# tarepan/VectorQuantizedCPC

Hardware: AMD Instinct MI355X
Metric: audio samples/sec (WaveRNN-style decode, convert.py path: encode + generate) (higher is better)
Workload: dtype f32

## Files before the change

### vectorquantizedcpc_amd/csrc/scan.hip

```cpp
#include "common.h"
#include "ar_shared.h"
#include <math.h>

__global__ void build_wfrag_kernel(const float *__restrict__ W, int ldw, float *__restrict__ Wf, int n_rg,
                                   int K, int ksplit, int rowmode, int H) {
    const int SW = K / 16 / ksplit;
    const size_t total = (size_t)n_rg * ksplit * SW * 64;
    const size_t id = (size_t)blockIdx.x * blockDim.x + threadIdx.x;
    if (id >= total) return;
    const int lane = (int)(id & 63);
    size_t r = id >> 6;
    const int s = (int)(r % SW); r /= SW;
    const int w = (int)(r % ksplit);
    const int rg = (int)(r / ksplit);
    const int i = lane & 15, kq = lane >> 4, S = w * SW + s;
    int row;
    if (rowmode == 0) row = 16 * rg + i;
    else if (rowmode == 8) row = i < 8 ? 8 * rg + i : -1;
    else if (rowmode == 16) row = (rg % 3) * H + 16 * (rg / 3) + i;
    else row = (i >> 2) < rowmode ? (i >> 2) * H + 4 * rg + (i & 3) : -1;
    float4 v = make_float4(0.f, 0.f, 0.f, 0.f);
    if (row >= 0) v = *(const float4 *)(W + (size_t)row * ldw + 16 * S + 4 * kq);
    ((float4 *)Wf)[id] = v;
}
// ... 56 lines not shown
    float4 wf[SW];
    load_wfrag<SW>(p.Wf + (size_t)dir * (H / 4) * (H / 16) * 64 * 4, rg, 4, wave, lane, wf);
    const f32x4 acc = mv16<SW>(wf, hin, H, bt, wave, lane);
    const float v = reduce4(red, acc, wave, lane, tid);
    gate[tid >> 4][tid & 15] = v;
    __syncthreads();
    if (act) {
        float hn;
        if (G == 3) {
            const float r = sigmoidf_(g0 + (gate[u][b] + bh0));
            const float z = sigmoidf_(g1 + (gate[4 + u][b] + bh1));
            const float n = tanhf(g2 + r * (gate[8 + u][b] + bh2));
            hn = (1.0f - z) * n + z * hold;
        } else {
            const float ig = sigmoidf_(g0 + gate[u][b]), fg = sigmoidf_(g1 + gate[4 + u][b]);
            const float gg = tanhf(g2 + gate[8 + u][b]), og = sigmoidf_(g3 + gate[12 + u][b]);
            const float cn = fg * cold + ig * gg;
            p.cbuf[(size_t)dir * hsz + hi] = cn;
            hn = og * tanhf(cn);
        }
        hout[hi] = hn;
        p.out[((p.row0 ? (size_t)p.row0[bg] : (size_t)bg * p.T) + tpos) * (p.ndir * H) + (size_t)dir * H + unit] = hn;
    }
}

template <int G>
static int launch_seq(const SeqP &p, int step, hipStream_t s) {
    const int SW = p.H / 64;
    dim3 grid(p.H / 4, p.ndir, p.nbt), blk(256);
    switch (SW) {
#define CASE(n) case n: hipLaunchKernelGGL((seq_step_kernel<G, n>), grid, blk, 0, s, p, step); break;
        CASE(1) CASE(2) CASE(4) CASE(8)
#undef CASE
        default: vq_set_error("recurrent step: hidden size %d unsupported (64, 128, 256 and 512 are built)", p.H); return VQCPC_ERR_INVALID;
    }
    return VQCPC_OK;
}

int vq_bigru_scan(const float *Wf, const float *b_hh, const float *Gi, float *hbuf, float *out, const int *len, const int *row0,
                  int H, int B, int T, hipStream_t s) {
    const int nbt = (B + 15) / 16;
    HIP_TRY(hipMemsetAsync(hbuf, 0, (size_t)2 * 2 * nbt * H * 16 * sizeof(float), s));
    SeqP q{};
    q.Wf = Wf; q.b_hh = b_hh; q.Gi = Gi; q.hbuf = hbuf;
    q.out = out; q.len = len; q.row0 = row0; q.H = H; q.nbt = nbt; q.B = B; q.T = T; q.ndir = 2;
    for (int t = 0; t < T; ++t) TRY(launch_seq<3>(q, t, s));
    return VQCPC_OK;
}

__global__ void add_vec_kernel(const float *a, const float *b, float *o, int n) {
    const int i = blockIdx.x * blockDim.x + threadIdx.x;
    if (i < n) o[i] = a[i] + b[i];
}

struct LstmPlan {
    int D, H;
    float *w_ih = nullptr, *bias = nullptr, *Wf = nullptr;
    float *w_hh = nullptr;
    DevBuf gi, hbuf, cbuf, px;
    unsigned *abort_host = nullptr;
    int persistent = -1;
    bool pending = false;
    int dbg_drop_step = -1;
    int timeout_ms = 1000;
};
static int lstm_persist_launch(LstmPlan *p, int T, float *out, hipStream_t s);
void vq_lstm_plan_destroy(LstmPlan *p) {
    if (!p) return;
    if (p->w_ih) (void)hipFree(p->w_ih);
    if (p->bias) (void)hipFree(p->bias);
    if (p->Wf) (void)hipFree(p->Wf);
    if (p->w_hh) (void)hipFree(p->w_hh);
    if (p->abort_host) (void)hipHostFree(p->abort_host);
    p->gi.release(); p->hbuf.release(); p->cbuf.release(); p->px.release();
    delete p;
}
int vq_lstm_plan_create(const float *w_ih, const float *w_hh, const float *b_ih, const float *b_hh, int D, int H,
                        LstmPlan **out) {
    VQ_REQUIRE(D % 32 == 0 && (H == 64 || H == 128 || H == 256 || H == 512), "LSTM: need D %% 32 == 0 and a hidden size of 64, 128, 256 "
               "(model.py:57) or 512 (got %d, %d)", D, H);
    LstmPlan *p = new LstmPlan();
    p->D = D; p->H = H;
    *out = p;
    HIP_TRY(hipMalloc((void **)&p->w_ih, (size_t)4 * H * D * sizeof(float)));
    HIP_TRY(hipMemcpy(p->w_ih, w_ih, (size_t)4 * H * D * sizeof(float), hipMemcpyDeviceToDevice));
    HIP_TRY(hipMalloc((void **)&p->bias, (size_t)4 * H * sizeof(float)));
    hipLaunchKernelGGL(add_vec_kernel, dim3((4 * H + 255) / 256), dim3(256), 0, 0, b_ih, b_hh, p->bias, 4 * H);
    HIP_TRY(hipGetLastError());
    TRY(vq_build_wfrag(w_hh, H, H / 4, H, 4, 4, H, &p->Wf));
    HIP_TRY(hipMalloc((void **)&p->w_hh, (size_t)4 * H * H * sizeof(float)));
    HIP_TRY(hipMemcpy(p->w_hh, w_hh, (size_t)4 * H * H * sizeof(float), hipMemcpyDeviceToDevice));
    HIP_TRY(hipHostMalloc((void **)&p->abort_host, 64, hipHostMallocMapped));
    *p->abort_host = 0u;
    return VQCPC_OK;
}
int vq_lstm_set_persistent(LstmPlan *p, int value) { p->persistent = value; return VQCPC_OK; }
int vq_lstm_set_debug(LstmPlan *p, int drop_step, int timeout_ms) { p->dbg_drop_step = drop_step; p->timeout_ms = timeout_ms; return VQCPC_OK; }
int vq_lstm_check(LstmPlan *p) {
    if (!p->pending) return VQCPC_OK;
    p->pending = false;
    if (*(volatile unsigned *)p->abort_host != 0u) {
        *p->abort_host = 0u;
        p->persistent = 0;
        vq_set_error("encoder LSTM: an in-kernel exchange of the resident scan timed out (the context of that call is incomplete); "
                     "this handle now uses one launch per time step -- call again");
        return VQCPC_ERR_HIP;
    }
    return VQCPC_OK;
}
int vq_lstm_run(LstmPlan *p, const float *x, int B, int T, float *out, hipStream_t s) {
    const int H = p->H, nbt = (B + 15) / 16;
    TRY(p->gi.reserve((size_t)B * T * 4 * H * sizeof(float)));
    const size_t hsz = (size_t)nbt * H * 16 * sizeof(float);
    TRY(p->hbuf.reserve(2 * hsz));
    TRY(p->cbuf.reserve(hsz));
    TRY(vq_gemm_chain(x, p->D, p->w_ih, p->bias, p->gi.as<float>(), 4 * H, B * T, 4 * H, p->D, p->D, s));
    TRY(vq_lstm_check(p));
    if (p->persistent != 0 && B == 1 && H == 256 && T >= 1) return lstm_persist_launch(p, T, out, s);
    HIP_TRY(hipMemsetAsync(p->hbuf.p, 0, 2 * hsz, s));
    HIP_TRY(hipMemsetAsync(p->cbuf.p, 0, hsz, s));
    SeqP q{};
    q.Wf = p->Wf; q.Gi = p->gi.as<float>(); q.hbuf = p->hbuf.as<float>(); q.cbuf = p->cbuf.as<float>();
    q.out = out; q.len = nullptr; q.H = H; q.nbt = nbt; q.B = B; q.T = T; q.ndir = 1;
    for (int t = 0; t < T; ++t) TRY(launch_seq<4>(q, t, s));
    HIP_TRY(hipGetLastError());
    return VQCPC_OK;
}

__device__ __forceinline__ int ps_perm(int k) { return (k & ~15) | ((k & 3) << 2) | ((k >> 2) & 3); }

template <int NS>
__device__ __forceinline__ float ps_chain(const float (&w)[8 * NS], const float4 *hb, int kw, int c0) {
    float acc = 0.f;
#pragma unroll
    for (int s = 0; s < NS; ++s) {
        const float4 h0 = hb[(kw * NS + s) * 4 + c0], h1 = hb[(kw * NS + s) * 4 + c0 + 2];
        acc = __builtin_fmaf(w[8 * s + 0], h0.x, acc); acc = __builtin_fmaf(w[8 * s + 1], h0.y, acc);
        acc = __builtin_fmaf(w[8 * s + 2], h0.z, acc); acc = __builtin_fmaf(w[8 * s + 3], h0.w, acc);
        acc = __builtin_fmaf(w[8 * s + 4], h1.x, acc); acc = __builtin_fmaf(w[8 * s + 5], h1.y, acc);
        acc = __builtin_fmaf(w[8 * s + 6], h1.z, acc); acc = __builtin_fmaf(w[8 * s + 7], h1.w, acc);
    }
    return acc;
}
__device__ __forceinline__ float ps_combine(float acc, int lane) {
    (void)lane;
    const float other = PS_DPP(acc, 0xB1);
    const float q = acc + other;
    const float q1 = PS_DPP(q, 0x4E);
    const float q2 = PS_DPP(q, 0x104);
    const float q3 = PS_DPP(q, 0x106);
    return ((q + q1) + q2) + q3;
}

#define PS_PAD 16
__device__ __forceinline__ int ps_slot(int idx, int per_blk) { return (idx / per_blk) * PS_PAD + idx % per_blk; }

template <int N>
__device__ __forceinline__ bool ps_sweep(const u64 *g, int lane, int per_blk, unsigned tag, unsigned (&val)[N], unsigned *abort_flag,
                                         u64 ticks = 100000000ull) {
    const u64 t0 = __builtin_amdgcn_s_memrealtime();
    int slot[N];
#pragma unroll
    for (int j = 0; j < N; ++j) slot[j] = ps_slot(lane + 64 * j, per_blk);
    for (unsigned spins = 0;; ++spins) {
        bool ok = true;
#pragma unroll
        for (int j = 0; j < N; ++j) {
            const u64 x = ps_load(g + slot[j]);
            val[j] = (unsigned)x;
            ok &= (unsigned)(x >> 32) == tag;
        }
        if (__all(ok)) return true;
        if ((spins & 63) == 63) {
            const bool late = __builtin_amdgcn_s_memrealtime() - t0 > ticks;
            if (late || __hip_atomic_load(abort_flag, __ATOMIC_RELAXED, __HIP_MEMORY_SCOPE_SYSTEM) != 0u) {
                if (late && lane == 0) __hip_atomic_store(abort_flag, 1u, __ATOMIC_RELAXED, __HIP_MEMORY_SCOPE_SYSTEM);
                return false;
            }
        }
        __builtin_amdgcn_s_sleep(1);
    }
}

#define LP_NW 32
#define LP_UPB 8
struct LstmPersistP {
    const float *w_hh;
    const float *Gi;
    float *out;
    u64 *g;
    unsigned *abort_flag;
    int T;
    int force_agent;
    int dbg_drop_step;
    unsigned timeout_ticks;
};
template <bool LOCAL>
__device__ __forceinline__ void lp_store(u64 *p, u64 v) {
    if (LOCAL) asm volatile("global_store_dwordx2 %0, %1, off sc0" :: "v"(p), "v"(v) : "memory");
    else ps_store(p, v);
}
__global__ __launch_bounds__(256) void lstm_persist_kernel(LstmPersistP p) {
    constexpr int H = 256;
    if (blockIdx.x % 8 != 0) return;
    const int blk = blockIdx.x / 8, tid = threadIdx.x, lane = tid & 63, wave = tid >> 6;
    __shared__ __attribute__((aligned(16))) float hbuf[H];
    __shared__ float gsum[4 * LP_UPB];
    const int row_local = tid >> 3, gate = row_local / LP_UPB, ul = row_local % LP_UPB;
    const int kw = (lane & 7) >> 1, c0 = lane & 1;
    float w[8 * 4];
    ps_load_weights<4>(p.w_hh + (size_t)(gate * H + LP_UPB * blk + ul) * H, kw, c0, w);
    const int unit = LP_UPB * blk + (tid < LP_UPB ? tid : 0);
    const u64 *gw = p.g + (size_t)(8 * wave) * PS_PAD;
    unsigned xcc;
    asm volatile("s_getreg_b32 %0, hwreg(HW_REG_XCC_ID)" : "=s"(xcc));
    xcc &= 0xfu;
    if (tid == 0) ps_store(p.g + (size_t)blk * PS_PAD + 8, ((u64)0xC0DEu << 32) | xcc);
    bool dead = false, local = true;
    {
        const u64 t0 = __builtin_amdgcn_s_memrealtime();
        for (unsigned spins = 0;; ++spins) {
            const u64 x = ps_load(p.g + (size_t)(lane & 31) * PS_PAD + 8);
            if (__all((unsigned)(x >> 32) == 0xC0DEu)) { local = __all((unsigned)x == xcc) && !p.force_agent; break; }
            if ((spins & 63) == 63 && (__builtin_amdgcn_s_memrealtime() - t0 > 100000000ull ||
                                       __hip_atomic_load(p.abort_flag, __ATOMIC_RELAXED, __HIP_MEMORY_SCOPE_SYSTEM) != 0u)) {
                if (lane == 0) __hip_atomic_store(p.abort_flag, 1u, __ATOMIC_RELAXED, __HIP_MEMORY_SCOPE_SYSTEM);
                dead = true;
                break;
            }
            __builtin_amdgcn_s_sleep(1);
        }
    }
    float cst = 0.f;
    float gi0 = 0.f, gi1 = 0.f, gi2 = 0.f, gi3 = 0.f;
    if (tid < LP_UPB) { const float *gp = p.Gi + unit; gi0 = gp[0]; gi1 = gp[H]; gi2 = gp[2 * H]; gi3 = gp[3 * H]; }
    for (int t = 0; t < p.T; ++t) {
        float hv = 0.f;
        if (t > 0 && !dead) {
            unsigned v[1];
            if (ps_sweep<1>(gw + (size_t)((t - 1) & 1) * LP_NW * PS_PAD, lane, LP_UPB, (unsigned)t, v, p.abort_flag, (u64)p.timeout_ticks)) hv = __uint_as_float(v[0]);
            else dead = true;
        }
        hbuf[ps_perm(tid)] = hv;
        ps_barrier();
        const float acc = ps_chain<4>(w, (const float4 *)hbuf, kw, c0);
        const float v = ps_combine(acc, lane);
        if ((lane & 7) == 0) gsum[row_local] = v;
        ps_barrier();
        if (tid < LP_UPB) {
            const float ig = sigmoidf_(gi0 + gsum[tid]), fg = sigmoidf_(gi1 + gsum[LP_UPB + tid]);
            const float gg = tanhf(gi2 + gsum[2 * LP_UPB + tid]), og = sigmoidf_(gi3 + gsum[3 * LP_UPB + tid]);
            cst = fg * cst + ig * gg;
            const float hn = og * tanhf(cst);
            const u64 gr = ((u64)(unsigned)(t + 1) << 32) | __float_as_uint(hn);
            u64 *dst = p.g + ((size_t)(t & 1) * LP_NW + blk) * PS_PAD + tid;
            const bool drop = p.dbg_drop_step == t && blk == 3;
            if (drop) { }
            else if (local) lp_store<true>(dst, gr);
            else lp_store<false>(dst, gr);
            p.out[(size_t)t * H + unit] = hn;
            if (t + 1 < p.T) { const float *gp = p.Gi + (size_t)(t + 1) * 4 * H + unit; gi0 = gp[0]; gi1 = gp[H]; gi2 = gp[2 * H]; gi3 = gp[3 * H]; }
        }
    }
}
static int lstm_persist_launch(LstmPlan *p, int T, float *out, hipStream_t s) {
    const size_t bytes = (size_t)2 * LP_NW * PS_PAD * sizeof(u64);
    TRY(p->px.reserve(bytes));
    HIP_TRY(hipMemsetAsync(p->px.p, 0, bytes, s));
    LstmPersistP q{};
    q.w_hh = p->w_hh; q.Gi = p->gi.as<float>(); q.out = out; q.g = p->px.as<u64>(); q.T = T;
    q.force_agent = p->persistent == 2;
    q.dbg_drop_step = p->dbg_drop_step;
    q.timeout_ticks = (unsigned)p->timeout_ms * 100000u;
    HIP_TRY(hipHostGetDevicePointer((void **)&q.abort_flag, p->abort_host, 0));
    hipLaunchKernelGGL(lstm_persist_kernel, dim3(8 * LP_NW), dim3(256), 0, s, q);
    HIP_TRY(hipGetLastError());
    p->pending = true;
    return VQCPC_OK;
}
```

### vectorquantizedcpc_amd/csrc/vocoder_host.hip

```cpp
#include "vocoder_internal.h"
#include <math.h>
#include <stdio.h>
#include <limits.h>


__global__ void quads_build_kernel(const float *__restrict__ src, float4 *__restrict__ dst, int rows, int H) {
    const size_t id = (size_t)blockIdx.x * blockDim.x + threadIdx.x;
    if (id >= (size_t)rows * H) return;
    const int unit = (int)(id % H);
    const size_t row = id / H;
    const float *s = src + row * 3 * H + unit;
    dst[row * H + unit] = make_float4(s[0], s[H], s[2 * H], 0.f);
}

__global__ void glue_kernel(const int64_t *__restrict__ idx, const int64_t *__restrict__ spk,
                            const float *__restrict__ ce, const float *__restrict__ se, float *__restrict__ out,
                            int B, int Tc, int dz, int ds, int n_codes, int n_spk, unsigned *status, unsigned status_tag,
                            const int *__restrict__ frames, const int *__restrict__ row0) {
    const int F = dz + ds;
    size_t i = (size_t)blockIdx.x * blockDim.x + threadIdx.x;
    if (i >= (size_t)B * 2 * Tc * F) return;
    const int f = (int)(i % F);
    const size_t r = i / F;
    const int t2 = (int)(r % (2 * Tc)), b = (int)(r / (2 * Tc));
    if (row0) {
        if (t2 >= frames[b]) return;
        i = ((size_t)row0[b] + t2) * F + f;
    }
    if (f < dz) {
        long long z = idx[(size_t)b * Tc + t2 / 2];
        if ((z < 0 || z >= n_codes) && f == 0 && status) __hip_atomic_fetch_or(status, status_tag | STATUS_BAD_INDEX, __ATOMIC_RELAXED, __HIP_MEMORY_SCOPE_SYSTEM);
        z = z < 0 ? 0 : (z >= n_codes ? n_codes - 1 : z);
        out[i] = ce[(size_t)z * dz + f];
    } else {
        long long sp = spk[b];
        if ((sp < 0 || sp >= n_spk) && f == dz && t2 == 0 && status) __hip_atomic_fetch_or(status, status_tag | STATUS_BAD_INDEX, __ATOMIC_RELAXED, __HIP_MEMORY_SCOPE_SYSTEM);
        sp = sp < 0 ? 0 : (sp >= n_spk ? n_spk - 1 : sp);
        out[i] = se[(size_t)sp * ds + (f - dz)];
    }
}

__global__ void copy_submatrix_kernel(const float *__restrict__ src, int ld, int col0, float *__restrict__ dst,
                                      int rows, int cols) {
    const size_t i = (size_t)blockIdx.x * blockDim.x + threadIdx.x;
    if (i >= (size_t)rows * cols) return;
    const int r = (int)(i / cols), cidx = (int)(i % cols);
    dst[i] = src[(size_t)r * ld + col0 + cidx];
}
static ArStep step_of(vqcpc_vocoder *v) { return ArStep{v->d.Hr, v->d.Hf, v->d.n_cls, v->big_min_tiles, &v->big_attr_set}; }

static void clear_graphs(vqcpc_vocoder::Group &G) {
    for (auto &kv : G.graphs) (void)hipGraphExecDestroy(kv.second);
    G.graphs.clear();
}
static void clear_graphs(vqcpc_vocoder *v) {
    for (auto &G : v->grp) clear_graphs(G);
}

static std::vector<DevBuf *> device_buffers(vqcpc_vocoder *v, bool fixed) {
    std::vector<DevBuf *> b = {&v->series, &v->gi, &v->out0, &v->cond, &v->gcond, &v->gbase, &v->hseq, &v->len, &v->hall, &v->a1c, &v->nll_part, &v->nll_len,
                               &v->xd_x, &v->xd_segs};
    for (auto &G : v->grp) b.insert(b.end(), {&G.har, &G.a1, &G.cand_s, &G.cand_k, &G.slot_tab, &G.cur, &G.gcur, &G.candg});
    if (!fixed) return b;
    b.insert(b.end(), {&v->code_emb, &v->spk_emb, &v->w_cond, &v->b_ih, &v->Gemb, &v->Gemb4, &v->bh4, &v->Wf_hh12, &v->Wf_hh16, &v->b_hh, &v->Wf_fc1,
                       &v->Wf_fc1h, &v->b_fc1, &v->Wf_fc2, &v->b_fc2, &v->w_fc1, &v->w_fc2, &v->mulaw_tab, &v->w_hh, &v->grp[0].call, &v->grp[1].call});
    for (int l = 0; l < 2; ++l) b.insert(b.end(), {&v->p_wih[l], &v->p_bih[l], &v->p_bhh[l], &v->p_wf[l]});
    return b;
}

static int dcopy(DevBuf &dst, const float *src, size_t n) {
    TRY(dst.reserve(n * sizeof(float)));
    HIP_TRY(hipMemcpy(dst.p, src, n * sizeof(float), hipMemcpyDeviceToDevice));
    return VQCPC_OK;
}

extern "C" void vqcpc_vocoder_destroy(vqcpc_vocoder *v) {
    if (!v) return;
    clear_graphs(v);
    for (DevBuf *b : device_buffers(v, true)) b->release();
    v->stage.release();
    if (v->status_host) (void)hipHostFree(v->status_host);
    for (hipStream_t st : {v->side_stream, v->cap_stream}) if (st) (void)hipStreamDestroy(st);
    for (hipEvent_t e : {v->ev_fork, v->ev_join, v->ev0, v->ev1}) if (e) (void)hipEventDestroy(e);
    delete v;
}

static int vocoder_create_impl(const vqcpc_vocoder_weights *w, vqcpc_vocoder *v) {
    v->d = *w;
    const int F = w->dz + w->ds, Hp = w->Hp, dl = 2 * Hp, Hr = w->Hr, de = w->de;
    struct Temps { DevBuf w_emb, emb, frag; ~Temps() { w_emb.release(); emb.release(); frag.release(); } } tmp;
    TRY(dcopy(v->code_emb, w->code_embedding, (size_t)w->n_codes * w->dz));
    TRY(dcopy(v->spk_emb, w->speaker_embedding, (size_t)w->n_speakers * w->ds));
    for (int l = 0; l < 2; ++l) {
        const int I = l == 0 ? F : dl;
        TRY(v->p_wih[l].reserve((size_t)6 * Hp * I * sizeof(float)));
        TRY(v->p_bih[l].reserve((size_t)6 * Hp * sizeof(float)));
        TRY(v->p_bhh[l].reserve((size_t)6 * Hp * sizeof(float)));
        TRY(v->p_wf[l].reserve((size_t)2 * (Hp / 4) * (Hp / 16) * 64 * sizeof(float4)));
        for (int d = 0; d < 2; ++d) {
            HIP_TRY(hipMemcpy(v->p_wih[l] + (size_t)d * 3 * Hp * I, w->prenet_w_ih[l][d], (size_t)3 * Hp * I * sizeof(float), hipMemcpyDeviceToDevice));
            HIP_TRY(hipMemcpy(v->p_bih[l] + (size_t)d * 3 * Hp, w->prenet_b_ih[l][d], (size_t)3 * Hp * sizeof(float), hipMemcpyDeviceToDevice));
            HIP_TRY(hipMemcpy(v->p_bhh[l] + (size_t)d * 3 * Hp, w->prenet_b_hh[l][d], (size_t)3 * Hp * sizeof(float), hipMemcpyDeviceToDevice));
            TRY(vq_build_wfrag(w->prenet_w_hh[l][d], Hp, Hp / 4, Hp, 4, 3, Hp, tmp.frag.fresh<float>()));
            const size_t nb = (size_t)(Hp / 4) * (Hp / 16) * 64 * sizeof(float4);
            HIP_TRY(hipMemcpy((char *)v->p_wf[l].p + d * nb, tmp.frag.p, nb, hipMemcpyDeviceToDevice));
        }
    }
    TRY(tmp.w_emb.reserve((size_t)3 * Hr * de * sizeof(float)));
    TRY(v->w_cond.reserve((size_t)3 * Hr * dl * sizeof(float)));
    hipLaunchKernelGGL(copy_submatrix_kernel, dim3((unsigned)(((size_t)3 * Hr * de + 255) / 256)), dim3(256), 0, 0,
                       w->ar_w_ih, de + dl, 0, tmp.w_emb.as<float>(), 3 * Hr, de);
    hipLaunchKernelGGL(copy_submatrix_kernel, dim3((unsigned)(((size_t)3 * Hr * dl + 255) / 256)), dim3(256), 0, 0,
                       w->ar_w_ih, de + dl, de, v->w_cond.as<float>(), 3 * Hr, dl);
    HIP_TRY(hipGetLastError());
    TRY(dcopy(v->b_ih, w->ar_b_ih, (size_t)3 * Hr));
    TRY(dcopy(v->b_hh, w->ar_b_hh, (size_t)3 * Hr));
    TRY(v->Gemb.reserve((size_t)w->n_cls * 3 * Hr * sizeof(float)));
    TRY(dcopy(tmp.emb, w->ar_embedding, (size_t)w->n_cls * de));
    TRY(vq_gemm_chain(tmp.emb.as<float>(), de, tmp.w_emb.as<float>(), nullptr, v->Gemb, 3 * Hr, w->n_cls, 3 * Hr, de, de, 0));
    TRY(v->Gemb4.reserve((size_t)w->n_cls * Hr * sizeof(float4)));
    TRY(v->bh4.reserve((size_t)Hr * sizeof(float4)));
    hipLaunchKernelGGL(quads_build_kernel, dim3((unsigned)(((size_t)w->n_cls * Hr + 255) / 256)), dim3(256), 0, 0, v->Gemb.as<float>(), v->Gemb4.as<float4>(), w->n_cls, Hr);
    hipLaunchKernelGGL(quads_build_kernel, dim3((unsigned)((Hr + 255) / 256)), dim3(256), 0, 0, v->b_hh.as<float>(), v->bh4.as<float4>(), 1, Hr);
    HIP_TRY(hipGetLastError());
    TRY(build_wfrag12(w->ar_w_hh, Hr, Hr / 4, Hr, Hr, v->Wf_hh12.fresh<float>()));
    if (Hr % 16 == 0) TRY(vq_build_wfrag(w->ar_w_hh, Hr, 3 * (Hr / 16), Hr, 4, 16, Hr, v->Wf_hh16.fresh<float>()));
    TRY(vq_build_wfrag(w->fc1_weight, Hr, w->Hf / 16, Hr, 4, 0, 0, v->Wf_fc1.fresh<float>()));
    TRY(vq_build_wfrag(w->fc1_weight, Hr, w->Hf / 8, Hr, 4, 8, 0, v->Wf_fc1h.fresh<float>()));
    TRY(vq_build_wfrag(w->fc2_weight, w->Hf, w->n_cls / 16, w->Hf, 1, 0, 0, v->Wf_fc2.fresh<float>()));
    TRY(dcopy(v->w_hh, w->ar_w_hh, (size_t)3 * Hr * Hr));
    TRY(dcopy(v->w_fc1, w->fc1_weight, (size_t)w->Hf * Hr));
    TRY(dcopy(v->w_fc2, w->fc2_weight, (size_t)w->n_cls * w->Hf));
    TRY(dcopy(v->b_fc1, w->fc1_bias, w->Hf));
    TRY(dcopy(v->b_fc2, w->fc2_bias, w->n_cls));
    std::vector<float> tab(w->n_cls);
    const double mu = (double)((1 << w->bits_mu_law) - 1);
    for (int s = 0; s < w->n_cls; ++s) {
        const double y = 2.0 * (double)s / mu - 1.0, sg = (y > 0) - (y < 0);
        tab[s] = (float)(sg / mu * (pow(1.0 + mu, fabs(y)) - 1.0));
    }
    TRY(v->mulaw_tab.reserve(tab.size() * sizeof(float)));
    HIP_TRY(hipMemcpy(v->mulaw_tab, tab.data(), tab.size() * sizeof(float), hipMemcpyHostToDevice));
    for (auto &g : v->grp) TRY(g.call.reserve(sizeof(ArCall)));
    if (w->Hf == NLL_HF && w->n_cls == NLL_CLS) TRY(vq_tf_nll_prepare());
    HIP_TRY(hipHostMalloc((void **)&v->status_host, 64, hipHostMallocMapped));
    *v->status_host = 0u;
    HIP_TRY(hipHostGetDevicePointer((void **)&v->status_dev, v->status_host, 0));
    HIP_TRY(hipStreamCreateWithFlags(&v->side_stream, hipStreamNonBlocking));
    HIP_TRY(hipEventCreateWithFlags(&v->ev_fork, hipEventDisableTiming));
    HIP_TRY(hipEventCreateWithFlags(&v->ev_join, hipEventDisableTiming));
    HIP_TRY(hipStreamCreateWithFlags(&v->cap_stream, hipStreamNonBlocking));
    HIP_TRY(hipEventCreate(&v->ev0));
    HIP_TRY(hipEventCreate(&v->ev1));
    HIP_TRY(hipDeviceSynchronize());
    return VQCPC_OK;
}

extern "C" int vqcpc_vocoder_create(const vqcpc_vocoder_weights *w, vqcpc_vocoder **out) {
    VQ_REQUIRE(w && out, "vqcpc_vocoder_create: null argument");
    *out = nullptr;
    TRY(vq_require_gfx950());
    VQ_REQUIRE(w->bits_mu_law >= 8 && w->bits_mu_law <= 10 && w->n_cls == (1 << w->bits_mu_law),
               "vocoder: bits_mu_law must be 8 (config.py:15), 9 or 10 with n_cls = 2^bits (got %d, %d)", w->bits_mu_law, w->n_cls);
    VQ_REQUIRE(w->Hf >= 256 && w->Hf <= 1024 && w->Hf % 256 == 0, "vocoder: size_h_fc must be 256 (config.py:77), 512, 768 or 1024 (got %d)", w->Hf);
    VQ_REQUIRE((w->dz + w->ds) % 32 == 0 && w->Hp % 64 == 0 && w->Hp <= 1024, "vocoder: dz+ds %% 32 and Hp %% 64 required");
    VQ_REQUIRE(w->de % 32 == 0, "vocoder: size_i_embed_ar %% 32 required (got %d)", w->de);
    VQ_REQUIRE(w->Hr == 512 || w->Hr == 896 || w->Hr == 1024, "vocoder: size_h_rnn %d: the per-sample kernels are built for 512, 896 "
               "(config.py:76) and 1024", w->Hr);
    VQ_REQUIRE(w->Hp == 64 || w->Hp == 128 || w->Hp == 256 || w->Hp == 512, "vocoder: dim_voc_latent / 2 = %d: the prenet scan is built "
               "for 64, 128 (config.py:68), 256 and 512", w->Hp);
    VQ_REQUIRE(w->upsample_t > 0, "vocoder: upsample_t must be positive");
    vqcpc_vocoder *v = new vqcpc_vocoder();
    int rc = vocoder_create_impl(w, v);
    if (rc != VQCPC_OK) { vqcpc_vocoder_destroy(v); return rc; }
    *out = v;
    return VQCPC_OK;
}

enum { OPT_BOOL = 1, OPT_GRAPHS = 2, OPT_EVEN = 4 };
struct OptSpec { const char *name; int vqcpc_vocoder::*field; int lo, hi, flags; };
static const OptSpec k_options[] = {
    {"use_graph", &vqcpc_vocoder::use_graph, 0, 1, OPT_BOOL},
    {"steps_per_graph", &vqcpc_vocoder::steps_per_graph, 2, 4096, OPT_GRAPHS | OPT_EVEN},
    {"big_min_tiles", &vqcpc_vocoder::big_min_tiles, 0, INT_MAX, OPT_GRAPHS},
    {"two_groups", &vqcpc_vocoder::two_groups, 0, 1, OPT_BOOL},
    {"fuse_fc2", &vqcpc_vocoder::fuse_fc2, 0, 1, OPT_BOOL | OPT_GRAPHS},
    {"handoff_timeout_ms", &vqcpc_vocoder::handoff_timeout_ms, 1, 10000, OPT_GRAPHS},
    {"handoff_debug_drop_step", &vqcpc_vocoder::handoff_debug_drop_step, INT_MIN, INT_MAX, OPT_GRAPHS},
    {"xcd", &vqcpc_vocoder::xcd, -1, 1, 0},
    {"xcd_slots", &vqcpc_vocoder::xcd_slots, 1, 8 * XD_MAX_BX, 0},
    {"xcd_agent_stores", &vqcpc_vocoder::xcd_agent_stores, 0, 1, OPT_BOOL},
    {"xcm", &vqcpc_vocoder::xcm, -1, 1, 0},
    {"xcm_min", &vqcpc_vocoder::xcm_min, 0, 65536, 0},
    {"xcm_max", &vqcpc_vocoder::xcm_max, 0, 1 << 20, 0},
    {"xcm_slots", &vqcpc_vocoder::xcm_slots, 1, 8 * XM_BX, 0},
    {"xcd_timeout_ms", &vqcpc_vocoder::xcd_timeout_ms, 1, 10000, 0},
    {"xcd_debug_drop_step", &vqcpc_vocoder::xcd_debug_drop_step, INT_MIN, INT_MAX, 0},
    {"xcd_debug_misplace", &vqcpc_vocoder::xcd_debug_misplace, 0, 1, OPT_BOOL},
    {"tf_chunk_replays", &vqcpc_vocoder::tf_chunk_replays, 1, 64, 0},
    {"slots", &vqcpc_vocoder::n_slots, 0, 65536, 0},
};

extern "C" int vqcpc_vocoder_set_option(vqcpc_vocoder *v, const char *name, int value) {
    VQ_REQUIRE(v && name, "vqcpc_vocoder_set_option: null argument");
    for (const OptSpec &o : k_options) {
        if (strcmp(name, o.name)) continue;
        if (o.flags & OPT_BOOL) value = value != 0;
        VQ_REQUIRE(value >= o.lo && value <= o.hi && !((o.flags & OPT_EVEN) && value % 2), "%s must be %sin [%d, %d]", name,
                   (o.flags & OPT_EVEN) ? "even and " : "", o.lo, o.hi);
        if ((o.flags & OPT_GRAPHS) && value != v->*o.field) clear_graphs(v);
        v->*o.field = value;
        if (o.field == &vqcpc_vocoder::xcd) { v->fell_back = false; v->placement_misses = 0; }
        return VQCPC_OK;
    }
    vq_set_error("unknown option %s", name);
    return VQCPC_ERR_INVALID;
}

constexpr int REARM_CLEAN = 16;
static void fall_back(vqcpc_vocoder *v) {
    if (!v->fell_back) { v->saved_xcd = v->xcd; v->saved_fuse_fc2 = v->fuse_fc2; }
    v->fell_back = true; v->clean_calls = 0; v->xcd = 0;
}
static int status_check(vqcpc_vocoder *v, bool synced) {
    if (!v->status_pending) return VQCPC_OK;
    const unsigned flag = *(volatile unsigned *)v->status_host;
    if (flag == 0) {
        if (synced) {
            v->status_pending = false;
            v->placement_misses = 0;
            if (v->fell_back && ++v->clean_calls >= REARM_CLEAN) {
                v->fell_back = false;
                v->xcd = v->saved_xcd;
                if (v->saved_fuse_fc2 && !v->fuse_fc2) { v->fuse_fc2 = 1; clear_graphs(v); }
            }
        }
        return VQCPC_OK;
    }
    *(volatile unsigned *)v->status_host = 0u;
    v->status_pending = false;
    const unsigned code = flag & 0xffu, ep = flag >> 8;
    char which[64];
    if (ep) snprintf(which, sizeof which, "call #%u of this handle", ep);
    else snprintf(which, sizeof which, "an earlier call of this handle");
    if (code & STATUS_BAD_INDEX) {
        vq_set_error("index out of range in self (%s): a code index or speaker id outside its embedding table (network_vocoder.py:73,75), "
                     "or a sample class outside [0, n_cls) in a scored position of vqcpc_vocoder_nll", which);
        return VQCPC_ERR_INVALID;
    }
    if (code & STATUS_MISPLACED) {
        v->placement_misses += 1;
        if (v->placement_misses >= 2) {
            fall_back(v);
            vq_set_error("decode not run (%s): the resident decoders' workgroups were not dealt 32 to each XCD, twice in a row (no output was "
                         "written; the GPU is probably shared) -- this handle now uses one launch per kernel and step; repeat the call", which);
        } else {
            vq_set_error("decode not run (%s): the resident decoders' workgroups were not dealt 32 to each XCD (no output was written; "
                         "another kernel held compute units) -- repeat the call", which);
        }
        return VQCPC_ERR_HIP;
    }
    fall_back(v);
    if (v->fuse_fc2) { v->fuse_fc2 = 0; clear_graphs(v); }
    vq_set_error("decode aborted (%s): an in-kernel exchange timed out (outputs of that call are incomplete); this handle now uses one launch "
                 "per kernel and step, and re-arms after %d clean calls or set_option xcd / fuse_fc2 -- repeat the call", which, REARM_CLEAN);
    return VQCPC_ERR_HIP;
}

extern "C" int vqcpc_vocoder_last_path(vqcpc_vocoder *v) {
    return v ? v->last_path : -1;
}

extern "C" int vqcpc_vocoder_check(vqcpc_vocoder *v) {
    VQ_REQUIRE(v, "vqcpc_vocoder_check: null argument");
    return status_check(v, true);
}

extern "C" int vqcpc_vocoder_last_slots(vqcpc_vocoder *v) {
    return v ? v->last_slots : -1;
}

extern "C" int vqcpc_vocoder_workspace_bytes(vqcpc_vocoder *v, uint64_t *bytes) {
    VQ_REQUIRE(v && bytes, "vqcpc_vocoder_workspace_bytes: null argument");
    uint64_t n = 0;
    for (DevBuf *b : device_buffers(v, false)) n += b->cap;
    *bytes = n;
    return VQCPC_OK;
}

extern "C" int vqcpc_vocoder_last_timing(vqcpc_vocoder *v, float *loop_ms, int *n_steps) {
    VQ_REQUIRE(v && loop_ms && n_steps, "vqcpc_vocoder_last_timing: null argument");
    TRY(status_check(v, true));
    HIP_TRY(hipEventElapsedTime(loop_ms, v->ev0, v->ev1));
    *n_steps = v->last_steps;
    return VQCPC_OK;
}

static int run_condition(vqcpc_vocoder *v, const int64_t *idx, const int64_t *spk, int B, int Tc,
                         const int *frames_dev, const int *row0_dev, size_t n_rows, float *cond_out, hipStream_t s) {
    const auto &d = v->d;
    const int F = d.dz + d.ds, Hp = d.Hp, dl = 2 * Hp, T2 = 2 * Tc, nbt = (B + 15) / 16;
    const size_t rows = row0_dev ? (n_rows ? n_rows : 1) : (size_t)B * T2;
    TRY(v->series.reserve(rows * F * sizeof(float)));
    TRY(v->gi.reserve(rows * 6 * Hp * sizeof(float)));
    TRY(v->out0.reserve(rows * dl * sizeof(float)));
    const size_t hsz = (size_t)2 * nbt * Hp * 16 * sizeof(float);
    TRY(v->hseq.reserve(2 * hsz));
    const size_t ng = (size_t)B * T2 * F;
    hipLaunchKernelGGL(glue_kernel, dim3((unsigned)((ng + 255) / 256)), dim3(256), 0, s, idx, spk, v->code_emb,
                       v->spk_emb, v->series.as<float>(), B, Tc, d.dz, d.ds, d.n_codes, d.n_speakers, v->status_dev, v->epoch << 8,
                       frames_dev, row0_dev);
    v->status_pending = true;
    for (int l = 0; l < 2; ++l) {
        const float *xin = l == 0 ? v->series.as<float>() : v->out0.as<float>();
        const int I = l == 0 ? F : dl;
        float *xout = l == 0 ? v->out0.as<float>() : cond_out;
        TRY(vq_gemm_chain(xin, I, v->p_wih[l], v->p_bih[l], v->gi.as<float>(), 6 * Hp, (int)rows, 6 * Hp, I, I, s));
        if (frames_dev && !row0_dev) HIP_TRY(hipMemsetAsync(xout, 0, rows * dl * sizeof(float), s));
        TRY(vq_bigru_scan(v->p_wf[l], v->p_bhh[l], v->gi.as<float>(), v->hseq.as<float>(), xout, frames_dev, row0_dev, Hp, B, T2, s));
    }
    HIP_TRY(hipGetLastError());
    return VQCPC_OK;
}

static int tf_chunk_gemms(vqcpc_vocoder *v, int B, int Ts, int CH, int chunk, float *logits, hipStream_t s) {
    const auto &d = v->d;
    const int M = B * CH;
    TRY(vq_gemm_chain_ex(v->hall.as<float>(), d.Hr, v->w_fc1, v->b_fc1, v->a1c.as<float>(), d.Hf, M, d.Hf, d.Hr, d.Hr,
                         1, 0, 0, 0, 0, s));
    TRY(vq_gemm_chain_ex(v->a1c.as<float>(), d.Hf, v->w_fc2, v->b_fc2, logits, d.n_cls, M, d.n_cls, d.Hf, d.Hf,
                         0, CH, Ts, chunk * CH, Ts, s));
    return VQCPC_OK;
}

struct NllCall {
    const int64_t *audio;
    int L;
    std::vector<int> slen;
    float *nll;
    double *nll_sum; int64_t *n_scored, *n_correct;
};

static int tf_chunk_nll(vqcpc_vocoder *v, int B, int CH, int chunk, const NllCall &nc, hipStream_t s) {
    NllHead h{};
    h.hall = v->hall.as<float>(); h.w1 = v->w_fc1; h.b1 = v->b_fc1; h.w2 = v->w_fc2; h.b2 = v->b_fc2;
    h.audio = nc.audio; h.slen = v->nll_len.as<int>(); h.nll = nc.nll; h.part = v->nll_part.as<NllPart>();
    h.status = v->status_dev; h.status_tag = v->epoch << 8;
    h.B = B; h.L = nc.L; h.CH = CH; h.t0 = chunk * CH; h.Hr = v->d.Hr;
    return vq_tf_nll_chunk(h, nc.nll_sum, nc.n_scored, nc.n_correct, s);
}
int run_resident(vqcpc_vocoder *v, const CallPlan &cp, int T2, unsigned long long seed, float *wav, int64_t *mulaw, hipStream_t s, const Resume *rs) {
    VQ_REQUIRE(!rs || cp.dp.path == 2, "vocoder stream: chunks do not run on the matrix-core decoders");
    const auto &d = v->d;
    const DecodePlan &pl = cp.dp;
    const int B = (int)cp.utt.size();
    size_t max_seg = 1;
    for (auto &l : pl.lists) max_seg = l.size() + 1 > max_seg ? l.size() + 1 : max_seg;
    std::vector<XdSeg> tab((size_t)8 * pl.bxt * max_seg, XdSeg{-1, 0, 0, 0u});
    XdParams xp{};
    for (int q = 0; q < pl.xs; ++q) {
        for (size_t i = 0; i < pl.lists[q].size(); ++i) tab[(size_t)q * max_seg + i] = pl.lists[q][i];
        const int x = q % 8;
        if (pl.xend[q] + 1 > xp.n_steps[x]) xp.n_steps[x] = (int)pl.xend[q] + 1;
    }
    const size_t tab_bytes = tab.size() * sizeof(XdSeg);
    TRY(v->xd_segs.reserve(tab_bytes + (size_t)B * sizeof(int)));
    TRY(v->stage.upload((char *)v->xd_segs.p + tab_bytes, cp.gbase.data(), (size_t)B * sizeof(int), s));
    TRY(v->xd_x.reserve(pl.path == 3 ? xm_exchange_bytes() : xd_exchange_bytes(pl.bxt)));
    TRY(v->stage.upload(v->xd_segs.p, tab.data(), tab_bytes, s));
    xp.w_hh = v->w_hh; xp.w_fc1 = v->w_fc1; xp.b_fc1 = v->b_fc1; xp.w_fc2 = v->w_fc2; xp.b_fc2 = v->b_fc2;
    xp.Gemb = v->Gemb; xp.b_hh = v->b_hh; xp.Gcond = v->gcond.as<float>(); xp.mulaw_tab = v->mulaw_tab;
    xp.segs = v->xd_segs.as<XdSeg>(); xp.xg = v->xd_x.as<unsigned long long>(); xp.status = v->status_dev;
    xp.status_tag = v->epoch << 8;
    xp.wav = wav; xp.mulaw = mulaw; xp.seed = seed; xp.max_seg = (int)max_seg; xp.n_slots = pl.xs; xp.bxt = pl.bxt;
    xp.Lout = d.upsample_t * T2; xp.F = T2; xp.upsample = d.upsample_t; xp.agent_stores = v->xcd_agent_stores;
    xp.timeout_ticks = (unsigned)v->xcd_timeout_ms * 100000u; xp.dbg_drop_step = v->xcd_debug_drop_step;
    xp.dbg_misplace = v->xcd_debug_misplace;
    if (rs) { xp.Lout = rs->Lout; xp.Gcond = rs->Gcond; }
    v->xcd_debug_misplace = 0;
    HIP_TRY(hipEventRecord(v->ev0, s));
    TRY(pl.path == 3 ? xm_launch(xp, s) : xd_launch(xp, s, rs ? &rs->x : nullptr));
    HIP_TRY(hipEventRecord(v->ev1, s));
    v->last_steps = (int)pl.longest;
    v->last_slots = pl.xs;
    v->last_path = pl.path;
    v->status_pending = true;
    return VQCPC_OK;
}

static int group_graph(vqcpc_vocoder *v, int g, const ArModel &m, int nbt, bool tf, hipGraphExec_t *out) {
    auto &G = v->grp[g];
    const void *now[8] = {G.har.p, G.a1.p, G.cand_s.p, G.cand_k.p, G.cur.p, G.gcur.p, G.candg.p, nullptr};
    if (memcmp(G.baked, now, sizeof now) != 0) {
        clear_graphs(G);
        memcpy(G.baked, now, sizeof now);
    }
    const int gkey = (((nbt * 17 + m.live_last) * 2 + m.lead6) * 2 + (tf ? 1 : 0)) * 3 + m.fused;
    auto it = G.graphs.find(gkey);
    if (it == G.graphs.end()) {
        hipGraph_t gr = nullptr;
        hipGraphExec_t ge = nullptr;
        HIP_TRY(hipStreamBeginCapture(v->cap_stream, hipStreamCaptureModeThreadLocal));
        int rc = launch_ar_steps(step_of(v), m, G.call, nbt, v->steps_per_graph, tf, v->cap_stream);
        hipError_t e = hipStreamEndCapture(v->cap_stream, &gr);
        if (rc != VQCPC_OK || e != hipSuccess) {
            if (gr) (void)hipGraphDestroy(gr);
            if (rc != VQCPC_OK) return rc;
            HIP_TRY(e);
        }
        e = hipGraphInstantiate(&ge, gr, nullptr, nullptr, 0);
        (void)hipGraphDestroy(gr);
        HIP_TRY(e);
        it = G.graphs.emplace(gkey, ge).first;
    }
    *out = it->second;
    return VQCPC_OK;
}

int run_launch_path(vqcpc_vocoder *v, const CallPlan &cp, const int64_t *inputs, int T2, int Ts, unsigned long long seed,
                    float *wav, int64_t *mulaw, float *logits, hipStream_t s, const Resume *rs, const NllCall *nc) {
    const auto &d = v->d;
    const int Hr = d.Hr, S = v->steps_per_graph, B = (int)cp.utt.size(), n_slots = cp.dp.xs, max_t = (int)cp.dp.longest;
    const bool tf = inputs != nullptr;
    ArCall calls[2];
    ArModel models[2];
    for (int g = 0; g < cp.n_grp; ++g) {
        auto &G = v->grp[g];
        const int nb = cp.tiles[g], Spg = nb * 16, slot0 = g * cp.tiles[0] * 16;
        const size_t tab_n = nc ? (size_t)Spg : cp.table[g].size();
        TRY(G.slot_tab.reserve(tab_n * sizeof(XdSeg)));
        TRY(G.cur.reserve((size_t)Spg * sizeof(XdSeg)));
        TRY(v->stage.upload(G.slot_tab.p, cp.table[g].data(), tab_n * sizeof(XdSeg), s));
        TRY(v->stage.upload(G.cur.p, cp.table[g].data(), (size_t)Spg * sizeof(XdSeg), s));
        const size_t hsz = (size_t)nb * Hr * 16 * sizeof(float);
        TRY(G.har.reserve(2 * hsz));
        TRY(G.a1.reserve((size_t)nb * d.Hf * 16 * sizeof(float)));
        const size_t nrg = (size_t)d.n_cls / 16;
        TRY(G.cand_s.reserve((size_t)Spg * nrg * sizeof(float)));
        TRY(G.cand_k.reserve((size_t)Spg * nrg * sizeof(int)));
        TRY(G.gcur.reserve((size_t)Spg * Hr * sizeof(float4)));
        HIP_TRY(hipMemsetAsync(G.har.p, 0, 2 * hsz, s));
        HIP_TRY(hipMemsetAsync(G.cand_s.p, 0, (size_t)Spg * nrg * sizeof(float), s));
        HIP_TRY(hipMemsetAsync(G.cand_k.p, 0, (size_t)Spg * nrg * sizeof(int), s));
        const size_t cg_bytes = (size_t)nb * nrg * 16 * sizeof(u64);
        TRY(G.candg.reserve(cg_bytes + 64));
        HIP_TRY(hipMemsetAsync(G.candg.p, 0, cg_bytes + 64, s));
        ArCall &c = calls[g];
        c = ArCall{};
        c.Gcond = v->gcond.as<float>(); c.gbase = v->gbase.as<int>(); c.inputs = inputs; c.wav = wav; c.mulaw = mulaw; c.logits = logits;
        c.slots = G.slot_tab.as<XdSeg>(); c.S = S; c.Sp = Spg; c.n_rep = cp.rep[g] > 0 ? cp.rep[g] : 1;
        c.F = T2; c.Ts = Ts; c.Lout = d.upsample_t * T2; c.max_t = cp.gmax[g]; c.nbt = nb; c.seed = seed; c.t_base = 0;
        if (rs) {
            c.Gcond = rs->Gcond; c.gbase = rs->gbase; c.Lout = rs->Lout;
            c.wav = wav ? (float *)((uintptr_t)wav - (uintptr_t)(rs->x.s0 - 1) * sizeof(float)) : nullptr;
            c.mulaw = mulaw ? (int64_t *)((uintptr_t)mulaw - (uintptr_t)(rs->x.s0 - 1) * sizeof(int64_t)) : nullptr;
            c.h_in = rs->x.s0 > 0 ? rs->x.h_in : nullptr; c.x_in = rs->x.x_in; c.h_out = rs->x.h_out; c.s0 = rs->x.s0;
        }
        if (tf) {
            c.CH = v->tf_chunk_replays * S;
            TRY(v->hall.reserve((size_t)B * c.CH * Hr * sizeof(float)));
            if (nc) {
                c.Ts = nc->L; c.one_row = 1;
                TRY(v->nll_part.reserve((size_t)B * vq_tf_nll_tiles(c.CH) * sizeof(NllPart)));
            } else TRY(v->a1c.reserve((size_t)B * c.CH * d.Hf * sizeof(float)));
            c.hall = v->hall.as<float>(); c.hall_t0 = 0;
            c.logits = nullptr;
        }
        TRY(v->stage.upload(G.call.p, &c, sizeof c, s));
        ArModel &m = models[g];
        m = ArModel{};
        m.Wf_hh12 = v->Wf_hh12; m.Wf_hh16 = v->Wf_hh16; m.bh4 = v->bh4; m.Gemb4 = v->Gemb4; m.Gemb = v->Gemb; m.Wf_fc1 = v->Wf_fc1; m.Wf_fc1h = v->Wf_fc1h; m.b_fc1 = v->b_fc1;
        m.Wf_fc2 = v->Wf_fc2; m.b_fc2 = v->b_fc2; m.mulaw_tab = v->mulaw_tab;
// ... 211 lines not shown
```

### vectorquantizedcpc_amd/csrc/vocoder_internal.h

```cpp
#pragma once
#include "common.h"
#include "ar_shared.h"
#include "ar_xcd.h"
#include "ar_step.h"
#include "nll.h"
#include <string.h>
#include <map>
#include <vector>

struct HostStage {
    char *p = nullptr;
    size_t cap = 0, used = 0;
    hipEvent_t ev = nullptr;
    bool pending = false;
    int begin(size_t need) {
        if (!ev) HIP_TRY(hipEventCreateWithFlags(&ev, hipEventDisableTiming));
        if (pending) { HIP_TRY(hipEventSynchronize(ev)); pending = false; }
        if (need > cap) {
            if (p) (void)hipHostFree(p);
            p = nullptr; cap = 0;
            const size_t want = need + need / 2 + 4096;
            HIP_TRY(hipHostMalloc((void **)&p, want, hipHostMallocDefault));
            cap = want;
        }
        used = 0;
        return VQCPC_OK;
    }
    int upload(void *dst, const void *src, size_t n, hipStream_t s) {
        const size_t at = (used + 15) & ~(size_t)15;
        VQ_REQUIRE(at + n <= cap, "host staging arena too small (%zu + %zu > %zu)", at, n, cap);
        memcpy(p + at, src, n);
        used = at + n;
        HIP_TRY(hipMemcpyAsync(dst, p + at, n, hipMemcpyHostToDevice, s));
        HIP_TRY(hipEventRecord(ev, s));
        pending = true;
        return VQCPC_OK;
    }
    void release() {
        if (pending && ev) (void)hipEventSynchronize(ev);
        if (p) (void)hipHostFree(p);
        if (ev) (void)hipEventDestroy(ev);
        p = nullptr; ev = nullptr; cap = 0; pending = false;
    }
};

constexpr int XCM_MIN_DEFAULT = 68, XCM_MAX_DEFAULT = 512, XCD_SLOTS_DEFAULT = 8 * XD_MAX_BX, XCM_SLOTS_DEFAULT = 8 * XM_BX;

struct vqcpc_vocoder {
    vqcpc_vocoder_weights d;
    DevPtr<float> code_emb, spk_emb;
    DevPtr<float> p_wih[2], p_bih[2], p_bhh[2], p_wf[2];
    DevPtr<float> w_cond, b_ih, Gemb;
    DevPtr<float4> Gemb4, bh4;
    DevPtr<float> Wf_hh12, Wf_hh16, b_hh, Wf_fc1, Wf_fc1h, b_fc1, Wf_fc2, b_fc2;
    DevPtr<float> w_fc1, w_fc2;
    DevPtr<float> mulaw_tab;
    struct Group {
        DevPtr<ArCall> call;
        DevBuf har, a1, cand_s, cand_k, slot_tab, cur, gcur, candg;
        std::map<int, hipGraphExec_t> graphs;
        const void *baked[8] = {nullptr, nullptr, nullptr, nullptr, nullptr, nullptr, nullptr, nullptr};
    } grp[2];
    int two_groups = 1;
    hipStream_t side_stream = nullptr;
    hipEvent_t ev_fork = nullptr, ev_join = nullptr;
    DevBuf series, gi, out0, cond, gcond, gbase, hseq, len;
    DevBuf hall, a1c;
    DevBuf nll_part, nll_len;
    unsigned *status_host = nullptr;
    unsigned *status_dev = nullptr;
    HostStage stage;
    DevPtr<float> w_hh;
    int fuse_fc2 = 1;
    bool status_pending = false;
    unsigned epoch = 0;
    int last_slots = 0;
    int placement_misses = 0;
    bool fell_back = false;
    int saved_xcd = -1, saved_fuse_fc2 = 1, clean_calls = 0;
    int handoff_timeout_ms = 250;
    int handoff_debug_drop_step = -1;
    int xcd = -1;
    int xcd_slots = XCD_SLOTS_DEFAULT;
    int xcd_agent_stores = 0;
    int xcd_timeout_ms = 250;
    int xcd_debug_drop_step = -1;
    int xcm = -1;
    int xcm_min = XCM_MIN_DEFAULT, xcm_max = XCM_MAX_DEFAULT;
    int xcm_slots = XCM_SLOTS_DEFAULT;
    int xcd_debug_misplace = 0;
    DevBuf xd_x, xd_segs;
    int tf_chunk_replays = 4;
    int use_graph = 1, steps_per_graph = 160;
    int n_slots = 0;
    int big_min_tiles = 5;
    bool big_attr_set = false;
    hipStream_t cap_stream = nullptr;
    hipEvent_t ev0 = nullptr, ev1 = nullptr;
    int last_steps = 0;
    ArCall last_call{};
    ArModel last_model{};
    int last_path = 1;
};


struct PlanOpts {
    int xcd, xcm, xcm_min, xcm_max, xcd_slots, xcm_slots, n_slots; bool supported;
    int upsample_t, steps_per_graph, fuse_fc2, big_min_tiles, two_groups, use_graph;
};

struct DecodePlan {
    int path = 0, xs = 0, bxt = 0;
    long longest = 0;
    std::vector<std::vector<XdSeg>> lists;
    std::vector<long> xend;
};

struct UttLayout {
    std::vector<int> lens;
    std::vector<unsigned> utt;
    std::vector<int> gbase;
    long grows = 0;
};

struct CallPlan : UttLayout {
    DecodePlan dp;
    int n_grp = 1, tiles[2] = {0, 0}, rep[2] = {0, 0}, gmax[2] = {0, 0};
    std::vector<XdSeg> table[2];
};

std::vector<int> longest_first(const int *samples, int B);
int utt_layout(int B, int Tc, const int *n_codes_host, int upsample_t, unsigned utt_base, const uint32_t *utt_ids_host, UttLayout &u);
bool plan_decode(const PlanOpts &o, const int *samples, const unsigned *utt, const std::vector<int> &order, DecodePlan &pl);
int plan_call(const PlanOpts &o, int B, int Tc, const int *n_codes_host, bool tf, int Ts, int max_steps, unsigned utt_base, const uint32_t *utt_ids_host, CallPlan &cp, const int *tf_len = nullptr);
int plan_launch_tables(const PlanOpts &o, const int *samples, const std::vector<int> &order, bool tf, int B, int s0, CallPlan &cp);

struct Resume { XdResume x; int Lout; const float *Gcond; const int *gbase; };
struct NllCall;

PlanOpts plan_opts(const vqcpc_vocoder *v);
int begin_call(vqcpc_vocoder *v, const CallPlan &cp, int B);
int run_conditioning(vqcpc_vocoder *v, const UttLayout &u, const int64_t *idx, const int64_t *spk, int B, int Tc, DevBuf &cond, DevBuf &gcond, DevBuf &gbase, hipStream_t s);
int run_resident(vqcpc_vocoder *v, const CallPlan &cp, int T2, unsigned long long seed, float *wav, int64_t *mulaw, hipStream_t s, const Resume *rs = nullptr);
int run_launch_path(vqcpc_vocoder *v, const CallPlan &cp, const int64_t *inputs, int T2, int Ts, unsigned long long seed, float *wav, int64_t *mulaw, float *logits, hipStream_t s, const Resume *rs = nullptr, const NllCall *nc = nullptr);
```

Baseline: 9.060 million.

## Add register-resident bidirectional GRU scan kernel for prenet conditioning

Result: no change. 9.127 million (median of 6 runs) (+0.7%).

```diff
diff --git a/vectorquantizedcpc_amd/csrc/scan.hip b/vectorquantizedcpc_amd/csrc/scan.hip
--- a/vectorquantizedcpc_amd/csrc/scan.hip
+++ b/vectorquantizedcpc_amd/csrc/scan.hip
@@ -232,6 +232,79 @@
     return ((q + q1) + q2) + q3;
 }
 
+struct BigruResP {
+    const float *w_hh;
+    const float *b_hh;
+    const float *Gi;
+    float *out;
+    const int *len, *row0;
+    int T;
+};
+template <int NS>
+__global__ __launch_bounds__(512 * NS) void bigru_resident_kernel(BigruResP p) {
+    constexpr int H = 64 * NS;
+    __shared__ __attribute__((aligned(16))) float hb[2][H];
+    __shared__ float gsum[3][H];
+    const int b = blockIdx.x, dir = blockIdx.y, tid = threadIdx.x, lane = tid & 63;
+    const int L = p.len ? p.len[b] : p.T;
+    const int n_steps = L < p.T ? L : p.T;
+    if (n_steps <= 0) return;
+    const int unit = tid >> 3, kw = (lane & 7) >> 1, c0 = lane & 1;
+    float w[3][8 * NS];
+#pragma unroll
+    for (int g = 0; g < 3; ++g) ps_load_weights<NS>(p.w_hh + ((size_t)(dir * 3 + g) * H + unit) * H, kw, c0, w[g]);
+    const bool cell = tid < H;
+    const size_t row_base = p.row0 ? (size_t)p.row0[b] : (size_t)b * p.T;
+    const float *gi_base = p.Gi + (size_t)dir * 3 * H + (cell ? tid : 0);
+    float *out_base = p.out + (size_t)dir * H + (cell ? tid : 0);
+    float g0 = 0.f, g1 = 0.f, g2 = 0.f, bh0 = 0.f, bh1 = 0.f, bh2 = 0.f, hold = 0.f;
+    if (cell) {
+        const float *bh = p.b_hh + (size_t)dir * 3 * H + tid;
+        bh0 = bh[0]; bh1 = bh[H]; bh2 = bh[2 * H];
+        const float *gi = gi_base + (row_base + (dir == 0 ? 0 : L - 1)) * (6 * H);
+        g0 = gi[0]; g1 = gi[H]; g2 = gi[2 * H];
+        hb[0][ps_perm(tid)] = 0.f;
+    }
+    __builtin_amdgcn_s_waitcnt(0x0F70);
+    __syncthreads();
+    for (int step = 0; step < n_steps; ++step) {
+        float n0, n1, n2;
+        if (cell) {
+            const int nx = step + 1 < n_steps ? step + 1 : step;
+            const float *gi = gi_base + (row_base + (dir == 0 ? nx : L - 1 - nx)) * (6 * H);
+            n0 = gi[0]; n1 = gi[H]; n2 = gi[2 * H];
+        }
+        const float4 *hc = (const float4 *)hb[step & 1];
+        const float s0 = ps_combine(ps_chain<NS>(w[0], hc, kw, c0), lane);
+        const float s1 = ps_combine(ps_chain<NS>(w[1], hc, kw, c0), lane);
+        const float s2 = ps_combine(ps_chain<NS>(w[2], hc, kw, c0), lane);
+        if ((lane & 7) == 0) { gsum[0][unit] = s0; gsum[1][unit] = s1; gsum[2][unit] = s2; }
+        __syncthreads();
+        if (cell) {
+            const float r = sigmoidf_(g0 + (gsum[0][tid] + bh0));
+            const float z = sigmoidf_(g1 + (gsum[1][tid] + bh1));
+            const float n = tanhf(g2 + r * (gsum[2][tid] + bh2));
+            const float hn = (1.0f - z) * n + z * hold;
+            hb[(step + 1) & 1][ps_perm(tid)] = hn;
+            out_base[(row_base + (dir == 0 ? step : L - 1 - step)) * (2 * H)] = hn;
+            hold = hn;
+            g0 = n0; g1 = n1; g2 = n2;
+        }
+        __syncthreads();
+    }
+}
+bool vq_bigru_resident_fits(int H) { return H == 64 || H == 128; }
+int vq_bigru_scan(const float *Wf, const float *w_hh, const float *b_hh, const float *Gi, float *hbuf, float *out, const int *len,
+                  const int *row0, int H, int B, int T, int resident, hipStream_t s) {
+    if (!resident || !vq_bigru_resident_fits(H)) return vq_bigru_scan(Wf, b_hh, Gi, hbuf, out, len, row0, H, B, T, s);
+    if (T <= 0) return VQCPC_OK;
+    const BigruResP q{w_hh, b_hh, Gi, out, len, row0, T};
+    if (H == 64) hipLaunchKernelGGL(bigru_resident_kernel<1>, dim3(B, 2), dim3(512), 0, s, q);
+    else hipLaunchKernelGGL(bigru_resident_kernel<2>, dim3(B, 2), dim3(1024), 0, s, q);
+    HIP_TRY(hipGetLastError());
+    return VQCPC_OK;
+}
+
 #define PS_PAD 16
 __device__ __forceinline__ int ps_slot(int idx, int per_blk) { return (idx / per_blk) * PS_PAD + idx % per_blk; }
 
diff --git a/vectorquantizedcpc_amd/csrc/vocoder_host.hip b/vectorquantizedcpc_amd/csrc/vocoder_host.hip
--- a/vectorquantizedcpc_amd/csrc/vocoder_host.hip
+++ b/vectorquantizedcpc_amd/csrc/vocoder_host.hip
@@ -64,7 +64,7 @@
     if (!fixed) return b;
     b.insert(b.end(), {&v->code_emb, &v->spk_emb, &v->w_cond, &v->b_ih, &v->Gemb, &v->Gemb4, &v->bh4, &v->Wf_hh12, &v->Wf_hh16, &v->b_hh, &v->Wf_fc1,
                        &v->Wf_fc1h, &v->b_fc1, &v->Wf_fc2, &v->b_fc2, &v->w_fc1, &v->w_fc2, &v->mulaw_tab, &v->w_hh, &v->grp[0].call, &v->grp[1].call});
-    for (int l = 0; l < 2; ++l) b.insert(b.end(), {&v->p_wih[l], &v->p_bih[l], &v->p_bhh[l], &v->p_wf[l]});
+    for (int l = 0; l < 2; ++l) b.insert(b.end(), {&v->p_wih[l], &v->p_bih[l], &v->p_bhh[l], &v->p_wf[l], &v->p_whh[l]});
     return b;
 }
 
@@ -97,10 +97,12 @@
         TRY(v->p_bih[l].reserve((size_t)6 * Hp * sizeof(float)));
         TRY(v->p_bhh[l].reserve((size_t)6 * Hp * sizeof(float)));
         TRY(v->p_wf[l].reserve((size_t)2 * (Hp / 4) * (Hp / 16) * 64 * sizeof(float4)));
+        TRY(v->p_whh[l].reserve((size_t)6 * Hp * Hp * sizeof(float)));
         for (int d = 0; d < 2; ++d) {
             HIP_TRY(hipMemcpy(v->p_wih[l] + (size_t)d * 3 * Hp * I, w->prenet_w_ih[l][d], (size_t)3 * Hp * I * sizeof(float), hipMemcpyDeviceToDevice));
             HIP_TRY(hipMemcpy(v->p_bih[l] + (size_t)d * 3 * Hp, w->prenet_b_ih[l][d], (size_t)3 * Hp * sizeof(float), hipMemcpyDeviceToDevice));
             HIP_TRY(hipMemcpy(v->p_bhh[l] + (size_t)d * 3 * Hp, w->prenet_b_hh[l][d], (size_t)3 * Hp * sizeof(float), hipMemcpyDeviceToDevice));
+            HIP_TRY(hipMemcpy(v->p_whh[l] + (size_t)d * 3 * Hp * Hp, w->prenet_w_hh[l][d], (size_t)3 * Hp * Hp * sizeof(float), hipMemcpyDeviceToDevice));
             TRY(vq_build_wfrag(w->prenet_w_hh[l][d], Hp, Hp / 4, Hp, 4, 3, Hp, tmp.frag.fresh<float>()));
             const size_t nb = (size_t)(Hp / 4) * (Hp / 16) * 64 * sizeof(float4);
             HIP_TRY(hipMemcpy((char *)v->p_wf[l].p + d * nb, tmp.frag.p, nb, hipMemcpyDeviceToDevice));
@@ -188,6 +190,7 @@
     {"handoff_timeout_ms", &vqcpc_vocoder::handoff_timeout_ms, 1, 10000, OPT_GRAPHS},
     {"handoff_debug_drop_step", &vqcpc_vocoder::handoff_debug_drop_step, INT_MIN, INT_MAX, OPT_GRAPHS},
     {"xcd", &vqcpc_vocoder::xcd, -1, 1, 0},
+    {"prenet_resident", &vqcpc_vocoder::prenet_resident, -1, 1, 0},
     {"xcd_slots", &vqcpc_vocoder::xcd_slots, 1, 8 * XD_MAX_BX, 0},
     {"xcd_agent_stores", &vqcpc_vocoder::xcd_agent_stores, 0, 1, OPT_BOOL},
     {"xcm", &vqcpc_vocoder::xcm, -1, 1, 0},
@@ -296,6 +299,8 @@
     return VQCPC_OK;
 }
 
+static bool prenet_resident(const vqcpc_vocoder *v) { return v->prenet_resident != 0 && vq_bigru_resident_fits(v->d.Hp); }
+
 static int run_condition(vqcpc_vocoder *v, const int64_t *idx, const int64_t *spk, int B, int Tc,
                          const int *frames_dev, const int *row0_dev, size_t n_rows, float *cond_out, hipStream_t s) {
     const auto &d = v->d;
@@ -304,8 +309,9 @@
     TRY(v->series.reserve(rows * F * sizeof(float)));
     TRY(v->gi.reserve(rows * 6 * Hp * sizeof(float)));
     TRY(v->out0.reserve(rows * dl * sizeof(float)));
+    const bool resident = prenet_resident(v);
     const size_t hsz = (size_t)2 * nbt * Hp * 16 * sizeof(float);
-    TRY(v->hseq.reserve(2 * hsz));
+    if (!resident) TRY(v->hseq.reserve(2 * hsz));
     const size_t ng = (size_t)B * T2 * F;
     hipLaunchKernelGGL(glue_kernel, dim3((unsigned)((ng + 255) / 256)), dim3(256), 0, s, idx, spk, v->code_emb,
                        v->spk_emb, v->series.as<float>(), B, Tc, d.dz, d.ds, d.n_codes, d.n_speakers, v->status_dev, v->epoch << 8,
@@ -317,7 +323,7 @@
         float *xout = l == 0 ? v->out0.as<float>() : cond_out;
         TRY(vq_gemm_chain(xin, I, v->p_wih[l], v->p_bih[l], v->gi.as<float>(), 6 * Hp, (int)rows, 6 * Hp, I, I, s));
         if (frames_dev && !row0_dev) HIP_TRY(hipMemsetAsync(xout, 0, rows * dl * sizeof(float), s));
-        TRY(vq_bigru_scan(v->p_wf[l], v->p_bhh[l], v->gi.as<float>(), v->hseq.as<float>(), xout, frames_dev, row0_dev, Hp, B, T2, s));
+        TRY(vq_bigru_scan(v->p_wf[l], v->p_whh[l], v->p_bhh[l], v->gi.as<float>(), v->hseq.as<float>(), xout, frames_dev, row0_dev, Hp, B, T2, resident, s));
     }
     HIP_TRY(hipGetLastError());
     return VQCPC_OK;
diff --git a/vectorquantizedcpc_amd/csrc/vocoder_internal.h b/vectorquantizedcpc_amd/csrc/vocoder_internal.h
--- a/vectorquantizedcpc_amd/csrc/vocoder_internal.h
+++ b/vectorquantizedcpc_amd/csrc/vocoder_internal.h
@@ -50,6 +50,7 @@
     vqcpc_vocoder_weights d;
     DevPtr<float> code_emb, spk_emb;
     DevPtr<float> p_wih[2], p_bih[2], p_bhh[2], p_wf[2];
+    DevPtr<float> p_whh[2];
     DevPtr<float> w_cond, b_ih, Gemb;
     DevPtr<float4> Gemb4, bh4;
     DevPtr<float> Wf_hh12, Wf_hh16, b_hh, Wf_fc1, Wf_fc1h, b_fc1, Wf_fc2, b_fc2;
@@ -81,6 +82,7 @@
     int handoff_timeout_ms = 250;
     int handoff_debug_drop_step = -1;
     int xcd = -1;
+    int prenet_resident = -1;
     int xcd_slots = XCD_SLOTS_DEFAULT;
     int xcd_agent_stores = 0;
     int xcd_timeout_ms = 250;
@@ -138,6 +140,10 @@
 struct Resume { XdResume x; int Lout; const float *Gcond; const int *gbase; };
 struct NllCall;
 
+bool vq_bigru_resident_fits(int H);
+int vq_bigru_scan(const float *Wf, const float *w_hh, const float *b_hh, const float *Gi, float *hbuf, float *out, const int *len,
+                  const int *row0, int H, int B, int T, int resident, hipStream_t s);
+
 PlanOpts plan_opts(const vqcpc_vocoder *v);
 int begin_call(vqcpc_vocoder *v, const CallPlan &cp, int B);
 int run_conditioning(vqcpc_vocoder *v, const UttLayout &u, const int64_t *idx, const int64_t *spk, int B, int Tc, DevBuf &cond, DevBuf &gcond, DevBuf &gbase, hipStream_t s);
```
